# ruotianluo/ImageCaptioning.pytorch

Hardware: NVIDIA H100
Metric: captions/sec at beam=5 seq_len=20 (higher is better)
Workload: dtype f32 (fp32-grade: split-fp16 x3 tensor-core passes, fp32 accumulate)

## Files before the change

### imagecaptioning.pytorch_b200/csrc/beam.cu

```cuda
#include "common.cuh"
#include "kernels.cuh"

namespace capb200 {

namespace {

constexpr int MAXB = 16;

__device__ __forceinline__ double apply_penalty(int kind, float alpha, int length, double p) {
    if (kind == 1) return p / (pow(5.0 + length, (double)alpha) / pow(6.0, (double)alpha));
    if (kind == 2) return p / (double)length;
    return p;
}

__device__ __forceinline__ void select_step(const BeamState& s, int img, int t, int live, int kl, int row0, int hist0, const float* __restrict__ top_val,
                                            const int* __restrict__ top_idx, const int* pen, int n_pen, float lambda, int penalty_kind,
                                            float penalty_alpha, double* __restrict__ done_p) {
    const int lane = threadIdx.x;
    const int b = s.beam, T = s.T;
    const int ncand = live * kl;
    float cv[8];
    int cf[8];
#pragma unroll
    for (int u = 0; u < 8; ++u) {
// ... 74 lines not shown
            s.done_len[rec] = t + 1;
            s.done_raw[rec] = new_sum;
            done_p[rec] = apply_penalty(penalty_kind, penalty_alpha, t + 1, (double)new_sum);
            new_sum -= 1000.0f;
        }
        s.sums[(long)img * b + lane] = new_sum;
        s.tokens[(long)img * b + lane] = word;
        s.src_row[(long)img * b + lane] = row0 + parent;
    }
    if (lane == 0 && em != 0u) s.done_cnt[img] = cnt0 + __popc(em);
}

__global__ void __launch_bounds__(32) beam_step_kernel(BeamState s, int t, int live, const float* __restrict__ top_val,
                                                       const int* __restrict__ top_idx, int penalty_kind, float penalty_alpha,
                                                       double* __restrict__ done_p) {
    const int img = blockIdx.x;
    select_step(s, img, t, live, s.beam, img * live, img * live, top_val, top_idx, nullptr, 0, 0.f, penalty_kind, penalty_alpha, done_p);
}

__global__ void __launch_bounds__(32) diverse_beam_step_kernel(BeamState s, int G, int t, int k, const float* __restrict__ top_val,
                                                               const int* __restrict__ top_idx, float lambda, int rows_total, int penalty_kind,
                                                               float penalty_alpha, double* __restrict__ done_p) {
    const int i = blockIdx.x, lane = threadIdx.x;
    const int b = s.beam, T = s.T;
    __shared__ int sh_pen[MAXB];
    for (int g = 0; g < G && g <= t; ++g) {
        const int lt = t - g;
        if (lt >= T) continue;
        const int n_pen = g * b;
        __syncwarp();
        if (lane < n_pen) {
            const int pg = lane / b, j = lane - pg * b;
            const int last = min(t - pg, T - 1);
            const int* seq_pg = (last & 1) ? s.seq_a : s.seq_b;
            sh_pen[lane] = seq_pg[((long)(i * G + pg) * b + j) * T + lt];
        }
        __syncwarp();
        const int vimg = i * G + g;
        select_step(s, vimg, lt, lt == 0 ? 1 : b, k, vimg * b, g * rows_total + vimg * b, top_val, top_idx, sh_pen, n_pen, lambda, penalty_kind,
                    penalty_alpha, done_p);
    }
}

__global__ void __launch_bounds__(32) beam_finalize_kernel(BeamState s, int keep, const double* __restrict__ done_p, long long* __restrict__ out_seq,
                                                           int* __restrict__ out_len, float* __restrict__ out_p, float* __restrict__ out_raw,
                                                           int* __restrict__ out_hist) {
    const int img = blockIdx.x, lane = threadIdx.x;
    const int b = s.beam, T = s.T;
    const int cnt = s.done_cnt[img];
    const long base = (long)img * b * T;
    __shared__ unsigned char taken[MAXB * 64];
    for (int i = lane; i < cnt; i += 32) taken[i] = 0;
    __syncwarp();
    for (int k = 0; k < keep; ++k) {
        double bv = -INFINITY;
        int bi = 0x7fffffff;
        for (int i = lane; i < cnt; i += 32) {
            if (!taken[i]) {
                const double v = done_p[base + i];
                if (v > bv || (v == bv && i < bi)) { bv = v; bi = i; }
            }
// ... 16 lines not shown
            out_p[o] = (float)bv;
            out_raw[o] = s.done_raw[base + bi];
        }
        const int len = s.done_len[base + bi];
        for (int q = lane; q < T; q += 32) {
            out_seq[o * T + q] = (q < len) ? (long long)s.done_seq[(base + bi) * T + q] : 0;
            out_hist[o * T + q] = (q < len) ? s.done_hist[(base + bi) * T + q] : -1;
        }
        __syncwarp();
    }
}

__global__ void beam_edit_kernel(int rows, int k_in, int beam, int t, DecodeEdits ed, const int* __restrict__ prev_tokens,
                                 const float* __restrict__ val_in, const int* __restrict__ idx_in, float* __restrict__ val_out, int* __restrict__ idx_out,
                                 int first_beam, int first_group_rows, int first_group) {
    const int r = blockIdx.x * blockDim.x + threadIdx.x;
    if (r >= rows) return;
    if (first_beam > 0 && (r % first_beam) / first_group_rows == first_group) t = 0;
    float v[MAXB];
    int ix[MAXB];
    const int prev = (t > 0 && prev_tokens != nullptr) ? prev_tokens[r] : -1;
    bool prev_bad = false;
    if (t > 0 && ed.n_bad > 0)
        for (int i = 0; i < ed.n_bad; ++i) prev_bad |= (ed.bad[i] == prev);
    for (int k = 0; k < k_in; ++k) {
        float x = val_in[(long)r * k_in + k];
        const int w = idx_in[(long)r * k_in + k];
        if (ed.constraint && t > 0 && w == prev) x = -INFINITY;
        if (prev_bad && w == 0) x = -INFINITY;
        if (w == ed.unk_col) x -= 1000.0f;
        v[k] = x;
        ix[k] = w;
    }
    for (int j = 0; j < beam; ++j) {
        int best = j;
        for (int k = j + 1; k < k_in; ++k)
            if (v[k] > v[best] || (v[k] == v[best] && ix[k] < ix[best])) best = k;
        const float tv = v[j]; v[j] = v[best]; v[best] = tv;
        const int ti = ix[j]; ix[j] = ix[best]; ix[best] = ti;
        val_out[(long)r * beam + j] = v[j];
        idx_out[(long)r * beam + j] = ix[j];
    }
}

__global__ void scale_rows_kernel(float* __restrict__ x, long ld, int rows, int cols, float f, int skip_beam, int skip_group_rows, int skip_group) {
    const long total = (long)rows * cols;
    for (long i = blockIdx.x * (long)blockDim.x + threadIdx.x; i < total; i += (long)gridDim.x * blockDim.x) {
        const long r = i / cols, c = i % cols;
        if (skip_beam > 0 && (int)(r % skip_beam) / skip_group_rows == skip_group) continue;
        x[r * ld + c] *= f;
    }
}

__global__ void gather_rows_kernel(const float* __restrict__ slab, long step_stride, long ld_slab, const int* __restrict__ hist, int T, int V1,
                                   float* __restrict__ dst, const float2* __restrict__ stats, long stats_stride, const long long* __restrict__ seqs,
                                   DecodeEdits ed) {
    const long item = blockIdx.x;
    const int sidx = (int)(item % T);
    const int row = hist[item];
    float* d = dst + item * V1;
    if (row < 0) {
        for (int v = threadIdx.x; v < V1; v += blockDim.x) d[v] = 0.f;
        return;
    }
    auto apply_edits = [&]() {
        if (seqs == nullptr || !ed.any()) return;
        __syncthreads();
        if (threadIdx.x == 0) {
            const int prev = sidx > 0 ? (int)seqs[item - 1] : -1;
            if (ed.unk_col >= 0 && ed.unk_col < V1) d[ed.unk_col] -= 1000.0f;
            if (ed.constraint && prev >= 0 && prev < V1) d[prev] = -INFINITY;
// ... 35 lines not shown
        const float4* s4 = reinterpret_cast<const float4*>(src);
        float4* d4 = reinterpret_cast<float4*>(d);
        for (int v = threadIdx.x; v < V1 / 4; v += blockDim.x) d4[v] = __ldg(s4 + v);
    } else {
        for (int v = threadIdx.x; v < V1; v += blockDim.x) d[v] = src[v];
    }
    apply_edits();
}

}

int beam_edit_launch(int rows, int k_in, int beam, int t, const DecodeEdits& ed, const int* prev_tokens, const float* val_in, const int* idx_in,
                     float* val_out, int* idx_out, cudaStream_t stream, int first_beam, int first_group_rows, int first_group) {
    CAPB_REQUIRE(k_in >= beam && k_in <= MAXB, "beam_size + number of active decode edits must be <= 16");
    if (rows <= 0) return 0;
    beam_edit_kernel<<<cdiv(rows, 128), 128, 0, stream>>>(rows, k_in, beam, t, ed, prev_tokens, val_in, idx_in, val_out, idx_out, first_beam,
                                                          first_group_rows, first_group);
    CAPB_CHECK_CUDA(cudaGetLastError());
    return 0;
}

int scale_rows_launch(float* x, long ld, int rows, int cols, float factor, cudaStream_t stream, int skip_beam, int skip_group_rows, int skip_group) {
    if (rows <= 0 || cols <= 0) return 0;
    long blocks = ((long)rows * cols + 255) / 256;
    if (blocks > sm_count() * 16) blocks = sm_count() * 16;
    scale_rows_kernel<<<(int)blocks, 256, 0, stream>>>(x, ld, rows, cols, factor, skip_beam, skip_group_rows, skip_group);
    CAPB_CHECK_CUDA(cudaGetLastError());
    return 0;
}

int beam_step_launch(const BeamState& s, int t, int live, const float* top_val, const int* top_idx, int penalty_kind, float penalty_alpha,
                     cudaStream_t stream) {
    CAPB_REQUIRE(s.beam >= 1 && s.beam <= MAXB, "beam size 1..16");
    CAPB_REQUIRE(s.beam * s.T <= MAXB * 64, "beam*T record capacity");
    beam_step_kernel<<<s.B, 32, 0, stream>>>(s, t, live, top_val, top_idx, penalty_kind, penalty_alpha, s.done_p);
    CAPB_CHECK_CUDA(cudaGetLastError());
    return 0;
}

int diverse_beam_step_launch(const BeamState& s, int G, int t, int k, const float* top_val, const int* top_idx, float lambda, int rows_total,
                             int penalty_kind, float penalty_alpha, cudaStream_t stream) {
    CAPB_REQUIRE(G >= 2 && s.beam >= 1 && G * s.beam <= MAXB, "group_size * beams per group must be in 2..16");
    CAPB_REQUIRE(k >= s.beam && k <= MAXB && s.beam * k <= 256, "candidate list width");
    CAPB_REQUIRE(s.beam * s.T <= MAXB * 64, "beam*T record capacity");
    CAPB_REQUIRE(lambda >= 0.f, "diversity_lambda must be >= 0 (the candidate lists rely on the penalty only lowering values)");
    diverse_beam_step_kernel<<<s.B / G, 32, 0, stream>>>(s, G, t, k, top_val, top_idx, lambda, rows_total, penalty_kind, penalty_alpha, s.done_p);
    CAPB_CHECK_CUDA(cudaGetLastError());
    return 0;
}

int beam_finalize_launch(const BeamState& s, int keep, long long* out_seq, int* out_len, float* out_p, float* out_raw, int* out_hist,
                         cudaStream_t stream) {
    CAPB_REQUIRE(keep >= 1 && keep <= s.beam, "keep must be in 1..beam");
    beam_finalize_kernel<<<s.B, 32, 0, stream>>>(s, keep, s.done_p, out_seq, out_len, out_p, out_raw, out_hist);
    CAPB_CHECK_CUDA(cudaGetLastError());
    return 0;
}

int gather_logprob_rows_launch(const float* slab, long step_stride, long ld_slab, const int* hist, int nseq, int T, int V1, float* dst,
                               const float2* stats, long stats_stride, cudaStream_t stream, const long long* seqs, const DecodeEdits* ed) {
    if (nseq <= 0) return 0;
    gather_rows_kernel<<<nseq * T, 256, 0, stream>>>(slab, step_stride, ld_slab, hist, T, V1, dst, stats, stats_stride, seqs, ed ? *ed : DecodeEdits());
    CAPB_CHECK_CUDA(cudaGetLastError());
    return 0;
}

}
```

### imagecaptioning.pytorch_b200/csrc/common.cuh

```cuda
#pragma once
#include <atomic>
#include <cstdint>
#include <cstdio>
#include <cstring>
#include <string>
#include <cuda.h>
#include <cuda_fp16.h>
#include <cuda_runtime.h>

namespace capb200 {

void set_error(const std::string& msg);
#define CAPB_CHECK_CUDA(expr)                                                                          \
    do {                                                                                               \
        cudaError_t _e = (expr);                                                                       \
        if (_e != cudaSuccess) {                                                                       \
            capb200::set_error(std::string(#expr) + " failed: " + cudaGetErrorString(_e) + " at " +    \
                               __FILE__ + ":" + std::to_string(__LINE__));                            \
            return 1;                                                                                  \
        }                                                                                              \
    } while (0)
#define CAPB_REQUIRE(cond, msg)                                                                        \
    do {                                                                                               \
        if (!(cond)) {                                                                                 \
// ... 10 lines not shown
    if (cudaGetDevice(&dev) != cudaSuccess || dev < 0 || dev > 63) return true;
    const unsigned long long bit = 1ull << dev;
    return (mask.fetch_or(bit) & bit) == 0;
}

inline int sm_count() {
    static std::atomic<int> cache[64];
    int dev = 0;
    if (cudaGetDevice(&dev) != cudaSuccess || dev < 0 || dev > 63) dev = 0;
    int n = cache[dev].load();
    if (n == 0) {
        if (cudaDeviceGetAttribute(&n, cudaDevAttrMultiProcessorCount, dev) != cudaSuccess || n < 1) n = 132;
        cache[dev].store(n);
    }
    return n;
}

__device__ __forceinline__ void split_f32(float x, __half& hi, __half& lo) {
    hi = __float2half_rn(x);
    lo = __float2half_rn(x - __half2float(hi));
}

constexpr int kMaxSeg = 3;
struct GemmSeg {
    const float* A = nullptr;
    long lda = 0;
    const float* W = nullptr;
    long ldw = 0;
    const __half* A_hi = nullptr;
    const __half* A_lo = nullptr;
// ... 90 lines not shown
```

### imagecaptioning.pytorch_b200/csrc/engine_common.cuh

```cuda
#pragma once
#include <cstdio>
#include <cstdlib>
#include <cstring>

#include "../../include/capb200.h"
#include "common.cuh"
#include "kernels.cuh"
#include "nvtx.cuh"

struct capb200_cider_table {
    capb200::CiderTable* t = nullptr;
};

namespace capb200 {

struct Planes {
    __half* hi = nullptr;
    __half* lo = nullptr;
    long ld = 0;
};

struct Arena {
    char* base = nullptr;
    size_t off = 0;
// ... 235 lines not shown
            va.topk = edits ? k_in : beam; va.top_val = d.top_val; va.top_idx = d.top_idx;
            va.stats = d.slab_stats + (long)t * rows;
            if (vocab_step_launch(va, st)) return 1;
            const float* tv = d.top_val;
            const int* ti = d.top_idx;
            if (edits) {
                if (beam_edit_launch(nrows, k_in, beam, t, ed, d.tokens, d.top_val, d.top_idx, d.top_val_e, d.top_idx_e, st)) return 1;
                tv = d.top_val_e; ti = d.top_idx_e;
                *launches += 1;
            }
            if (beam_step_launch(s, t, live, tv, ti, penalty_kind, penalty_alpha, st)) return 1;
            *launches += 2;
        }
        return 0;
    };
    unsigned long long key[8] = {graph_key, (unsigned long long)B, (unsigned long long)beam, (unsigned long long)T, (unsigned long long)V1,
                                 (unsigned long long)penalty_kind, 0ull, (unsigned long long)reinterpret_cast<uintptr_t>(d.slab)};
    memcpy(&key[6], &penalty_alpha, sizeof(float));
    memcpy(reinterpret_cast<char*>(&key[6]) + 4, &temperature, sizeof(float));
    key[5] ^= ((unsigned long long)(ed.constraint & 1) << 8) ^ ((unsigned long long)(unsigned)(ed.unk_col + 1) << 16) ^ ((unsigned long long)ed.n_bad << 48);
    key[0] ^= (unsigned long long)reinterpret_cast<uintptr_t>(ed.bad) * 0x9E3779B97F4A7C15ull;
    d.last_edits = ed;
    d.last_stats = d.slab_stats;
    if (run_beam_loop(d, key, graph_key != 0, launches, st, run_loop)) return 1;
    CAPB_NVTX("capb200 beam finalize + log-prob rows");
    if (beam_finalize_launch(s, beam, d.rec_seq, d.rec_len, d.rec_p, d.rec_raw, d.rec_hist, st)) return 1;
    *launches += 1;
    if (keep == beam) {
        CAPB_CHECK_CUDA(cudaMemcpyAsync(seq, d.rec_seq, sizeof(long long) * B * beam * T, cudaMemcpyDeviceToDevice, st));
        if (seq_logprobs) {
            *launches += 1;
// ... 59 lines not shown
            va.topk = edits ? k_in : beam; va.top_val = d.top_val; va.top_idx = d.top_idx;
            va.stats = d.dbs_stats + (long)t * rows;
            if (vocab_step_launch(va, st)) return 1;
            const float* tv = d.top_val;
            const int* ti = d.top_idx;
            if (edits) {
                if (beam_edit_launch(rows, k_in, beam, t, ed, d.tokens, d.top_val, d.top_idx, d.top_val_e, d.top_idx_e, st, beam, bdash, t)) return 1;
                tv = d.top_val_e; ti = d.top_idx_e;
                *launches += 1;
            }
            if (diverse_beam_step_launch(s, G, t, beam, tv, ti, lambda, rows, penalty_kind, penalty_alpha, st)) return 1;
            *launches += 2;
        }
        return 0;
    };
    unsigned long long key[8] = {graph_key, (unsigned long long)B, (unsigned long long)beam, (unsigned long long)T, (unsigned long long)V1,
                                 (unsigned long long)penalty_kind, 0ull, (unsigned long long)reinterpret_cast<uintptr_t>(d.slab)};
    memcpy(&key[6], &penalty_alpha, sizeof(float));
    memcpy(reinterpret_cast<char*>(&key[6]) + 4, &temperature, sizeof(float));
    key[5] ^= ((unsigned long long)(ed.constraint & 1) << 8) ^ ((unsigned long long)(unsigned)(ed.unk_col + 1) << 16) ^ ((unsigned long long)ed.n_bad << 48);
    key[0] ^= (unsigned long long)reinterpret_cast<uintptr_t>(ed.bad) * 0x9E3779B97F4A7C15ull;
    unsigned lambda_bits = 0;
    memcpy(&lambda_bits, &lambda, sizeof(float));
    key[3] ^= (1ull << 63) ^ ((unsigned long long)G << 40);
    key[1] ^= (unsigned long long)lambda_bits << 32;
    key[4] ^= (unsigned long long)reinterpret_cast<uintptr_t>(d.dbs_stats) * 0x9E3779B97F4A7C15ull;
    key[2] ^= (unsigned long long)reinterpret_cast<uintptr_t>(d.dbs_done_cnt) << 8;
    if (run_beam_loop(d, key, graph_key != 0, launches, st, run_loop)) return 1;

    CAPB_NVTX("capb200 diverse beam finalize + log-prob rows");
    if (beam_finalize_launch(s, bdash, d.rec_seq, d.rec_len, d.rec_p, d.rec_raw, d.rec_hist, st)) return 1;
// ... 236 lines not shown
```

### imagecaptioning.pytorch_b200/csrc/gemm_tc.cu

```cuda
#include <cstdlib>
#include <cstring>

#include "common.cuh"
#include "ptx.cuh"

namespace capb200 {

namespace {

constexpr int BM = 128;
constexpr int BK = 64;
constexpr int kConsumers = 2;
constexpr int kThreads = 128 * (1 + kConsumers);

struct TcParams {
    CUtensorMap a_hi[kMaxSeg];
    CUtensorMap a_lo[kMaxSeg];
    CUtensorMap w_hi[kMaxSeg];
    CUtensorMap w_lo[kMaxSeg];
    int kblocks[kMaxSeg];
    int nseg;
    int M, N;
    float* C;
    long ldc;
// ... 360 lines not shown
    extern __shared__ uint8_t smem_raw[];
    uint8_t* smem = reinterpret_cast<uint8_t*>((reinterpret_cast<uintptr_t>(smem_raw) + 1023) & ~uintptr_t(1023));
    uint64_t* full_bar = reinterpret_cast<uint64_t*>(smem + Cfg::kStages * Cfg::kStageBytes);
    uint64_t* empty_bar = full_bar + Cfg::kStages;
    uint64_t* turn_bar = empty_bar + Cfg::kStages;

    const int wg = threadIdx.x >> 7;
    const int n_tiles = p.tiles_m * p.tiles_n;

    if (threadIdx.x == 0) {
        init_ring<PASSES>(p, full_bar, empty_bar, Cfg::kStages, 1);
        for (int c = 0; c < kConsumers; ++c) ptx::mbar_init(&turn_bar[c], 1);
        ptx::fence_mbar_init();
    }
    __syncthreads();
    if (threadIdx.x == 0) CAPB_TRACE(0);

    if (wg == 0) {
        ptx::setmaxnreg_dec<40>();
        if (threadIdx.x == 0) {
            int stage = 0;
            uint32_t phase = 0;
            for (int t = blockIdx.x; t < n_tiles; t += gridDim.x) {
                const int m0 = (t % p.tiles_m) * BM;
                const int n0 = (t / p.tiles_m) * BN;
                for (int s = 0; s < p.nseg; ++s) {
                    for (int kb = 0; kb < p.kblocks[s]; ++kb) {
                        ptx::mbar_wait(&empty_bar[stage], phase ^ 1);
                        fill_stage<Cfg>(p, smem + stage * Cfg::kStageBytes, &full_bar[stage], s, kb, m0, n0);
                        if (++stage == Cfg::kStages) { stage = 0; phase ^= 1; }
// ... 44 lines not shown
__global__ void __launch_bounds__(kThreads, 1) gemm_tc256_kernel(const __grid_constant__ TcParams p) {
    using Cfg = TcCfg<BN, PASSES, 2 * BM>;
    extern __shared__ uint8_t smem_raw[];
    uint8_t* smem = reinterpret_cast<uint8_t*>((reinterpret_cast<uintptr_t>(smem_raw) + 1023) & ~uintptr_t(1023));
    uint64_t* full_bar = reinterpret_cast<uint64_t*>(smem + Cfg::kStages * Cfg::kStageBytes);
    uint64_t* empty_bar = full_bar + Cfg::kStages;

    const int wg = threadIdx.x >> 7;
    const int n_tiles = p.tiles_m * p.tiles_n;

    if (threadIdx.x == 0) {
        init_ring<PASSES>(p, full_bar, empty_bar, Cfg::kStages, kConsumers);
        ptx::fence_mbar_init();
    }
    __syncthreads();
    if (threadIdx.x == 0) CAPB_TRACE(0);

    if (wg == 0) {
        ptx::setmaxnreg_dec<40>();
        if (threadIdx.x == 0) {
            int stage = 0;
            uint32_t phase = 0;
            for (int t = blockIdx.x; t < n_tiles; t += gridDim.x) {
                const int m0 = (t % p.tiles_m) * Cfg::kTileM;
                const int n0 = (t / p.tiles_m) * BN;
                for (int s = 0; s < p.nseg; ++s) {
                    for (int kb = 0; kb < p.kblocks[s]; ++kb) {
                        ptx::mbar_wait(&empty_bar[stage], phase ^ 1);
                        fill_stage<Cfg>(p, smem + stage * Cfg::kStageBytes, &full_bar[stage], s, kb, m0, n0);
                        if (++stage == Cfg::kStages) { stage = 0; phase ^= 1; }
// ... 69 lines not shown
template <int BN, int PASSES, int EPI, bool TRACE, int TM>
int launch_cfg(const TcParams& prm, cudaStream_t stream) {
    using Cfg = TcCfg<BN, PASSES, TM>;
    void (*kernel)(TcParams);
    if constexpr (TM == BM) kernel = gemm_tc_kernel<BN, PASSES, EPI, TRACE>;
    else kernel = gemm_tc256_kernel<BN, PASSES, EPI, TRACE>;
    static std::atomic<unsigned long long> attr_set{0};
    if (first_use_on_device(attr_set)) {
        CAPB_CHECK_CUDA(cudaFuncSetAttribute(kernel, cudaFuncAttributeMaxDynamicSharedMemorySize, Cfg::kSmemBytes));
    }
    TcParams prm2 = prm;
    prm2.tiles_n = cdiv(prm.N, BN);
    prm2.tiles_m = cdiv(prm.M, TM);
    const int n_tiles = prm2.tiles_n * prm2.tiles_m;
    const int sms = sm_count();
    kernel<<<n_tiles < sms ? n_tiles : sms, kThreads, Cfg::kSmemBytes, stream>>>(prm2);
    CAPB_CHECK_CUDA(cudaGetLastError());
    return 0;
}

template <int EPI, int TM>
int launch_width(int bn, int passes, const TcParams& prm, cudaStream_t stream) {
    if (prm.trace != nullptr) {
        if (bn == 160) return launch_cfg<160, 3, EPI, true, TM>(prm, stream);
        if constexpr (TM == BM) if (bn == 64) return launch_cfg<64, 3, EPI, true, TM>(prm, stream);
        return launch_cfg<128, 3, EPI, true, TM>(prm, stream);
    }
    if (bn == 160) return passes == 3 ? launch_cfg<160, 3, EPI, false, TM>(prm, stream) : launch_cfg<160, 1, EPI, false, TM>(prm, stream);
    if constexpr (TM == BM) {
        if (bn == 64) return passes == 3 ? launch_cfg<64, 3, EPI, false, TM>(prm, stream) : launch_cfg<64, 1, EPI, false, TM>(prm, stream);
    }
    return passes == 3 ? launch_cfg<128, 3, EPI, false, TM>(prm, stream) : launch_cfg<128, 1, EPI, false, TM>(prm, stream);
// ... 114 lines not shown
```

### imagecaptioning.pytorch_b200/csrc/pointwise.cu

```cuda
#include "common.cuh"
#include "kernels.cuh"

namespace capb200 {

static int pw_blocks(long total) {
    long b = (total + 255) / 256;
    return (int)(b > sm_count() * 8 ? sm_count() * 8 : b);
}

namespace {

__device__ __forceinline__ float sigmoidf_(float x) { return fast_sigmoid(x); }

__device__ __forceinline__ void store_act(const ActView& o, long row, int col, float v) {
    o.f[row * o.ld + col] = v;
    if (o.hi != nullptr) {
        __half h, l;
        split_f32(v, h, l);
        o.hi[row * o.ld + col] = h;
        o.lo[row * o.ld + col] = l;
    }
}

__global__ void state_gather_embed_kernel(int rows, const int* __restrict__ tokens, const int* __restrict__ src_row,
                                          const float* __restrict__ emb, long ld_emb, int E, int relu, ActView xt,
                                          int H, int nstate, StateCopy sc0, StateCopy sc1) {
    const int r = blockIdx.x;
    if (r >= rows) return;
    const int tok = tokens[r];
    const float* e = emb + (long)tok * ld_emb;
    for (int c = threadIdx.x; c < E; c += blockDim.x) {
        float v = __ldg(e + c);
        if (relu) v = fmaxf(v, 0.f);
        store_act(xt, r, c, v);
    }
    const int src = src_row ? src_row[r] : r;
    const bool vec = (H & 3) == 0 && (sc0.ld_src & 3) == 0 && (sc0.dst.ld & 3) == 0 && (nstate < 2 || ((sc1.ld_src & 3) == 0 && (sc1.dst.ld & 3) == 0));
    if (vec) {
        for (int c4 = threadIdx.x; c4 < (H >> 2); c4 += blockDim.x) {
            float4 v0 = make_float4(0.f, 0.f, 0.f, 0.f), v1 = v0;
            if (src >= 0) {
// ... 112 lines not shown
    extern __shared__ float s_ah[];
    constexpr int AP = NA * 32;
    float* s_w = s_ah + ATT_JB * AP;
    constexpr float kC = 2.885390081777927f;
    const int img = blockIdx.y;
    const int warp = threadIdx.x >> 5, lane = threadIdx.x & 31;
    const int r = blockIdx.x * ATT_SW + warp;
    const float alpha_b = __ldg(alpha_b_ptr);
    float pv[NA];
    const bool live = r < R;
    const float* pr = p_att + ((long)img * R + (live ? r : 0)) * ld_pa;
    for (int i = threadIdx.x; i < AP; i += ATT_SW * 32) s_w[i] = (i < A) ? __ldg(alpha_w + i) : 0.f;
    __syncthreads();
    float wsum = 0.f;
#pragma unroll
    for (int k = 0; k < NA; ++k) {
        const int a = (NA % 4 == 0) ? 128 * (k >> 2) + 4 * lane + (k & 3) : lane + 32 * k;
        pv[k] = (live && a < A) ? __ldg(pr + a) * kC : 0.f;
        wsum += s_w[a];
    }
    for (int j0 = 0; j0 < rpi; j0 += ATT_JB) {
        const int nj = min(ATT_JB, rpi - j0);
        __syncthreads();
        for (int i = threadIdx.x; i < nj * AP; i += ATT_SW * 32) {
            const int j = i / AP, a = i - j * AP;
            s_ah[i] = (a < A) ? att_h[((long)img * rpi + j0 + j) * ld_ah + a] * kC : 0.f;
        }
        __syncthreads();
        if (live) {
            float part[ATT_JB];
#pragma unroll
            for (int j = 0; j < ATT_JB; ++j) {
                part[j] = 0.f;
                if (j < nj) {
// ... 34 lines not shown
#pragma unroll
            for (int j = 0; j < ATT_JB; ++j) {
                float v = part[j];
#pragma unroll
                for (int o = 16; o > 0; o >>= 1) v += __shfl_xor_sync(0xffffffffu, v, o);
                if (lane == 0 && j < nj) score[((long)img * rpi + j0 + j) * R + r] = v + alpha_b;
            }
        }
    }
}

constexpr int ATT_CT = 256;
__global__ void __launch_bounds__(ATT_CT) att_combine_kernel(int rpi, int R, int H, const float* __restrict__ score, const float* __restrict__ att,
                                                             long ld_at, const float* __restrict__ mask, long ld_mask, ActView out,
                                                             float* __restrict__ alpha_out) {
    extern __shared__ float s_w[];
    const int img = blockIdx.x;
    const int c = blockIdx.y * ATT_CT + threadIdx.x;
    const int warp = threadIdx.x >> 5, lane = threadIdx.x & 31;
    for (int j0 = 0; j0 < rpi; j0 += ATT_JB) {
        const int nj = min(ATT_JB, rpi - j0);
        __syncthreads();
        if (warp < nj) {
            const float* sc = score + ((long)img * rpi + j0 + warp) * R;
            float* w = s_w + warp * R;
            float mx = -INFINITY;
            for (int r = lane; r < R; r += 32) mx = fmaxf(mx, sc[r]);
#pragma unroll
            for (int o = 16; o > 0; o >>= 1) mx = fmaxf(mx, __shfl_xor_sync(0xffffffffu, mx, o));
            float sum = 0.f;
// ... 42 lines not shown
        if (out_flat.hi) { __half h, l; split_f32(v, h, l); out_flat.hi[i] = h; out_flat.lo[i] = l; }
    }
}

}

int relu_copy_launch(const float* x, long n, ActView out_flat, cudaStream_t stream) {
    relu_copy_kernel<<<pw_blocks(n), 256, 0, stream>>>(x, n, out_flat);
    CAPB_CHECK_CUDA(cudaGetLastError());
    return 0;
}

int state_gather_embed_launch(int rows, const int* tokens, const int* src_row, const float* emb, long ld_emb, int E, int relu,
                              ActView xt, int H, int nstate, StateCopy sc0, StateCopy sc1, cudaStream_t stream) {
    if (rows <= 0) return 0;
    state_gather_embed_kernel<<<rows, 256, 0, stream>>>(rows, tokens, src_row, emb, ld_emb, E, relu, xt, H, nstate, sc0, sc1);
    CAPB_CHECK_CUDA(cudaGetLastError());
    return 0;
}


int lstm_pointwise_launch(int rows, int H, const float* gates, long ld_g, const int* src_row, const float* c_prev, long ld_cp,
                          float* c_out, long ld_co, ActView h_out, const float* gather_bias, long ld_gb, const int* gather_idx,
                          cudaStream_t stream) {
    if (rows <= 0) return 0;
    lstm_pointwise_kernel<<<pw_blocks((long)rows * H), 256, 0, stream>>>(rows, H, gates, ld_g, src_row, c_prev, ld_cp, c_out, ld_co, h_out,
                                                                          gather_bias, ld_gb, gather_idx);
    CAPB_CHECK_CUDA(cudaGetLastError());
    return 0;
}

int lstm_ln_launch(int rows, int H, const float* gates, long ld_g, const float* c_prev, long ld_cp, float* c_out, long ld_co, float* h_out, long ld_h,
// ... 9 lines not shown
                            float* c_out, long ld_co, ActView h_out, cudaStream_t stream) {
    if (rows <= 0) return 0;
    maxout_pointwise_kernel<<<pw_blocks((long)rows * H), 256, 0, stream>>>(rows, H, sums, ld_s, src_row, c_prev, ld_cp, c_out, ld_co, h_out);
    CAPB_CHECK_CUDA(cudaGetLastError());
    return 0;
}

int additive_attention_launch(int n_images, int rpi, int R, int A, int H, const float* att_h, long ld_ah, const float* p_att, long ld_pa,
                              const float* att, long ld_at, const float* mask, long ld_mask, const float* alpha_w, const float* alpha_b,
                              float* score_scratch, ActView out, cudaStream_t stream, float* alpha_out) {
    if (n_images <= 0 || rpi <= 0) return 0;
    CAPB_REQUIRE(A <= 1024, "attention: att_hid_size above 1024");
    CAPB_REQUIRE(score_scratch != nullptr, "attention: score scratch missing");
    const int na = cdiv(A, 32);
    dim3 sgrid(cdiv(R, ATT_SW), n_images);
#define CAPB_ATT_CASE(NA_)                                                                                                             \
    att_score_kernel<NA_><<<sgrid, ATT_SW * 32, sizeof(float) * (ATT_JB + 1) * NA_ * 32, stream>>>(rpi, R, A, att_h, ld_ah, p_att, ld_pa, alpha_w, \
                                                                                               alpha_b, score_scratch)
    if (na <= 2) CAPB_ATT_CASE(2);
    else if (na <= 4) CAPB_ATT_CASE(4);
    else if (na <= 8) CAPB_ATT_CASE(8);
    else if (na <= 16) CAPB_ATT_CASE(16);
    else CAPB_ATT_CASE(32);
#undef CAPB_ATT_CASE
    CAPB_CHECK_CUDA(cudaGetLastError());
    const size_t smem = sizeof(float) * (size_t)ATT_JB * R;
    CAPB_REQUIRE(smem <= 48 * 1024, "attention: too many regions");
    dim3 grid(n_images, cdiv(H, ATT_CT));
    att_combine_kernel<<<grid, ATT_CT, smem, stream>>>(rpi, R, H, score_scratch, att, ld_at, mask, ld_mask, out, alpha_out);
    CAPB_CHECK_CUDA(cudaGetLastError());
    return 0;
}

}
```

### imagecaptioning.pytorch_b200/csrc/vocab.cu

```cuda
#include <cstdlib>

#include "common.cuh"
#include "kernels.cuh"
#include "ptx.cuh"

namespace capb200 {

static __device__ unsigned long long g_vocab_seed_salt = 0ull;
int dropout_salt_set_vocab(unsigned long long salt, cudaStream_t st) {
    return cudaMemcpyToSymbolAsync(g_vocab_seed_salt, &salt, sizeof(salt), 0, cudaMemcpyHostToDevice, st) == cudaSuccess ? 0 : 1;
}

namespace {

constexpr int VT = 256;

template <int NT = VT>
__device__ __forceinline__ float block_max(float v, float* scratch) {
#pragma unroll
    for (int o = 16; o > 0; o >>= 1) v = fmaxf(v, __shfl_xor_sync(0xffffffffu, v, o));
    __syncthreads();
    if ((threadIdx.x & 31) == 0) scratch[threadIdx.x >> 5] = v;
    __syncthreads();
    float r = scratch[0];
// ... 205 lines not shown
            }
            float ov;
            block_argmax<NT>(bv, bi, s_red, s_idx, ov, tok);
        }
        __syncthreads();
        if (threadIdx.x == 0) {
            if (a.unfinished) a.unfinished[r] = (tok != 0) ? 1 : 0;
            if (a.tokens_out) a.tokens_out[r] = tok;
            if (a.seq_out) a.seq_out[(long)r * a.ld_seq + a.t] = tok;
            if (a.picked_lp) a.picked_lp[(long)r * a.ld_picked] = row[tok];
        }
    }
}

__global__ void __launch_bounds__(VT) vocab_stats_kernel(const VocabStepArgs a) {
    __shared__ float s_red[VT / 32];
    __shared__ int s_idx[VT / 32];
    const int r = blockIdx.x;
    const int V1 = a.V1;
    const float* g = a.logits + (long)r * a.ld;
    const bool vec = ((V1 & 3) == 0) && ((a.ld & 3) == 0) && ((reinterpret_cast<uintptr_t>(a.logits) & 15) == 0);
    float mx = -INFINITY;
    if (vec) {
        const float4* g4 = reinterpret_cast<const float4*>(g);
        for (int v = threadIdx.x; v < V1 / 4; v += VT) { const float4 x = g4[v]; mx = fmaxf(mx, fmaxf(fmaxf(x.x, x.y), fmaxf(x.z, x.w))); }
    } else {
        for (int v = threadIdx.x; v < V1; v += VT) mx = fmaxf(mx, g[v]);
    }
    mx = block_max(mx, s_red);
    float t0v = -INFINITY, t1v = -INFINITY;
// ... 56 lines not shown
__device__ __forceinline__ void online_raise(float& part, float& m, float& mL, float m4) {
    const float nL = m4 * 1.4426950408889634f;
    float sc;
    asm("ex2.approx.ftz.f32 %0, %1;" : "=f"(sc) : "f"(mL - nL));
    part = (m == -INFINITY) ? 0.f : part * sc;
    m = m4;
    mL = nL;
}
__device__ __forceinline__ float online_finish(float part, float m, float mL, float mx) {
    float sc;
    asm("ex2.approx.ftz.f32 %0, %1;" : "=f"(sc) : "f"(fmaf(-mx, 1.4426950408889634f, mL)));
    return (m == -INFINITY) ? 0.f : part * sc;
}

__global__ void __launch_bounds__(VT) vocab_stats_online_kernel(const VocabStepArgs a) {
    __shared__ float s_red[VT / 32];
    __shared__ int s_idx[VT / 32];
    const int r = blockIdx.x;
    const int n4 = a.V1 >> 2;
    const float4* g4 = reinterpret_cast<const float4*>(a.logits + (long)r * a.ld);
    constexpr float kL2E = 1.4426950408889634f;
    float t0v = -INFINITY, t1v = -INFINITY;
    int t0i = 0x7fffffff, t1i = 0x7fffffff;
    float m = -INFINITY, mL = -INFINITY, part = 0.f;
    for (int v = threadIdx.x; v < n4; v += VT) {
        const float4 x = g4[v];
        const float m4 = fmaxf(fmaxf(x.x, x.y), fmaxf(x.z, x.w));
        if (m4 > m) {
            online_raise(part, m, mL, m4);
        }
// ... 75 lines not shown
    }
    __syncthreads();
    if ((threadIdx.x & 31) == 0) { sval[threadIdx.x >> 5] = v; sidx[threadIdx.x >> 5] = i; }
    __syncthreads();
    out_v = sval[0];
    out_i = sidx[0];
#pragma unroll
    for (int w = 1; w < VT2 / 32; ++w) {
        const float ov = sval[w];
        const int oi = sidx[w];
        if (ov > out_v || (ov == out_v && oi < out_i)) { out_v = ov; out_i = oi; }
    }
}

__global__ void __launch_bounds__(VT2) vocab_stats_online128_kernel(const VocabStepArgs a) {
    __shared__ float s_red[VT2 / 32];
    __shared__ int s_idx[VT2 / 32];
    const int r = blockIdx.x;
    const int n4 = a.V1 >> 2;
    const float4* g4 = reinterpret_cast<const float4*>(a.logits + (long)r * a.ld);
    constexpr float kL2E = 1.4426950408889634f;
    float t0v = -INFINITY, t1v = -INFINITY;
    int t0i = 0x7fffffff, t1i = 0x7fffffff;
    float m = -INFINITY, mL = -INFINITY, part = 0.f;
    auto consume = [&](const float4 x, int v) {
        const float m4 = fmaxf(fmaxf(x.x, x.y), fmaxf(x.z, x.w));
        if (m4 > m) {
            online_raise(part, m, mL, m4);
        }
        float e0, e1, e2, e3;
// ... 44 lines not shown
                    const float4 x = g4[w];
                    consider(x.x, 4 * w); consider(x.y, 4 * w + 1); consider(x.z, 4 * w + 2); consider(x.w, 4 * w + 3);
                }
            }
        }
        if (threadIdx.x == 0) {
            const float lp = (ov - mx) - lsum;
            a.top_val[(long)r * a.topk + k] = a.row_twice(r) ? (lp - m2) - l2 : lp;
            a.top_idx[(long)r * a.topk + k] = oi;
        }
    }
}

template <int NV>
__global__ void __launch_bounds__(VT) vocab_stats_reg_kernel(const VocabStepArgs a) {
    __shared__ float s_red[VT / 32];
    __shared__ int s_idx[VT / 32];
    const int r = blockIdx.x;
    const int n4 = a.V1 >> 2;
    const float4* g4 = reinterpret_cast<const float4*>(a.logits + (long)r * a.ld);
    float4 xs[NV];
#pragma unroll
    for (int i = 0; i < NV; ++i) {
        const int v = threadIdx.x + i * VT;
        xs[i] = v < n4 ? g4[v] : make_float4(-INFINITY, -INFINITY, -INFINITY, -INFINITY);
    }
    float mx = -INFINITY;
#pragma unroll
    for (int i = 0; i < NV; ++i) mx = fmaxf(mx, fmaxf(fmaxf(xs[i].x, xs[i].y), fmaxf(xs[i].z, xs[i].w)));
    mx = block_max(mx, s_red);
// ... 35 lines not shown
                for (int i = 0; i < NV; ++i) {
                    const int v = 4 * (threadIdx.x + i * VT);
                    if (v < a.V1) { consider(xs[i].x, v); consider(xs[i].y, v + 1); consider(xs[i].z, v + 2); consider(xs[i].w, v + 3); }
                }
            }
        }
        if (threadIdx.x == 0) {
            const float lp = (ov - mx) - lsum;
            a.top_val[(long)r * a.topk + k] = a.row_twice(r) ? (lp - m2) - l2 : lp;
            a.top_idx[(long)r * a.topk + k] = oi;
        }
    }
}

__global__ void __launch_bounds__(VT) vocab_stats_stream_kernel(const VocabStepArgs a) {
    extern __shared__ __align__(16) unsigned char vs_smem[];
    __shared__ float s_red[VT / 32];
    __shared__ int s_idx[VT / 32];
    __shared__ __align__(8) uint64_t bar[2];
    const int V1 = a.V1, n4 = V1 >> 2;
    const uint32_t row_bytes = (uint32_t)V1 * 4u;
    float* buf0 = reinterpret_cast<float*>(vs_smem);
    float* buf1 = buf0 + V1;
    if (threadIdx.x == 0) {
        ptx::mbar_init(&bar[0], 1);
        ptx::mbar_init(&bar[1], 1);
        ptx::fence_mbar_init();
    }
    __syncthreads();
    int r = blockIdx.x;
// ... 113 lines not shown
    }
}

}

int vocab_step_launch(const VocabStepArgs& a, cudaStream_t stream) {
    if (a.rows <= 0) return 0;
    CAPB_REQUIRE(a.topk <= 16, "beam size up to 16");
    if (a.stats != nullptr) {
        CAPB_REQUIRE(a.select == 0 && a.topk > 0, "stats mode is the beam-search epilogue");
        const bool vec = ((a.V1 & 3) == 0) && ((a.ld & 3) == 0) && ((reinterpret_cast<uintptr_t>(a.logits) & 15) == 0);
        const size_t stream_smem = sizeof(float) * 2 * (size_t)a.V1;
        static const char* variant = getenv("CAPB200_VOCAB_STATS");
        const char vsel = variant ? variant[0] : 'o';
        if (vec && vsel == 'o' && !(variant && variant[1] == '2')) {
            vocab_stats_online128_kernel<<<a.rows, VT2, 0, stream>>>(a);
        } else if (vec && vsel == 'o') {
            vocab_stats_online_kernel<<<a.rows, VT, 0, stream>>>(a);
        } else if (vec && vsel == 's' && stream_smem <= 100 * 1024) {
            static std::atomic<unsigned long long> configured{0};
            if (first_use_on_device(configured)) {
                CAPB_CHECK_CUDA(cudaFuncSetAttribute(vocab_stats_stream_kernel, cudaFuncAttributeMaxDynamicSharedMemorySize, (int)(100 * 1024)));
            }
            const int grid = a.rows < 2 * sm_count() ? a.rows : 2 * sm_count();
            vocab_stats_stream_kernel<<<grid, VT, stream_smem, stream>>>(a);
        } else if (vec && vsel == 'r' && a.V1 <= VT * 4 * 10) {
            vocab_stats_reg_kernel<10><<<a.rows, VT, 0, stream>>>(a);
        } else {
            vocab_stats_kernel<<<a.rows, VT, 0, stream>>>(a);
        }
        CAPB_CHECK_CUDA(cudaGetLastError());
        return 0;
    }
    const size_t smem = sizeof(float) * (size_t)a.V1;
    CAPB_REQUIRE(smem <= 200 * 1024, "vocabulary larger than 51200 entries needs the multi-pass variant");
    static std::atomic<unsigned long long> configured{0};
    if (first_use_on_device(configured)) {
        CAPB_CHECK_CUDA(cudaFuncSetAttribute(vocab_step_kernel<2>, cudaFuncAttributeMaxDynamicSharedMemorySize, (int)(200 * 1024)));
        CAPB_CHECK_CUDA(cudaFuncSetAttribute(vocab_step_kernel<8>, cudaFuncAttributeMaxDynamicSharedMemorySize, (int)(200 * 1024)));
        CAPB_CHECK_CUDA(cudaFuncSetAttribute(vocab_step_kernel<16>, cudaFuncAttributeMaxDynamicSharedMemorySize, (int)(200 * 1024)));
    }
    if (a.topk <= 2 && a.select != 0 && a.rows <= 2 * sm_count()) {
        static std::atomic<unsigned long long> configured2{0};
        if (first_use_on_device(configured2)) {
// ... 28 lines not shown
```

Before: 23870.

## Enable programmatic dependent launch across decode-step kernels

Launches the beam, attention, vocab, pointwise and GEMM kernels with the programmatic stream serialization attribute, adding griddepcontrol wait and launch-dependents calls at kernel entry. The next kernel's launch and prologue (barrier init, smem setup, attention weight sum) can then overlap the tail of the previous kernel in the many small per-step launches. The graph cache key now includes the PDL setting, and an environment variable can turn it off. The risk is a memory ordering error if a kernel touches predecessor outputs before its wait.

Result: faster. 24380, median of 6 (+2.1%).

```diff
diff --git a/imagecaptioning.pytorch_b200/csrc/beam.cu b/imagecaptioning.pytorch_b200/csrc/beam.cu
--- a/imagecaptioning.pytorch_b200/csrc/beam.cu
+++ b/imagecaptioning.pytorch_b200/csrc/beam.cu
@@ -112,6 +112,7 @@
 __global__ void __launch_bounds__(32) beam_step_kernel(BeamState s, int t, int live, const float* __restrict__ top_val,
                                                        const int* __restrict__ top_idx, int penalty_kind, float penalty_alpha,
                                                        double* __restrict__ done_p) {
+    pdl_enter();
     const int img = blockIdx.x;
     select_step(s, img, t, live, s.beam, img * live, img * live, top_val, top_idx, nullptr, 0, 0.f, penalty_kind, penalty_alpha, done_p);
 }
@@ -119,6 +120,7 @@
 __global__ void __launch_bounds__(32) diverse_beam_step_kernel(BeamState s, int G, int t, int k, const float* __restrict__ top_val,
                                                                const int* __restrict__ top_idx, float lambda, int rows_total, int penalty_kind,
                                                                float penalty_alpha, double* __restrict__ done_p) {
+    pdl_enter();
     const int i = blockIdx.x, lane = threadIdx.x;
     const int b = s.beam, T = s.T;
     __shared__ int sh_pen[MAXB];
@@ -143,6 +145,7 @@
 __global__ void __launch_bounds__(32) beam_finalize_kernel(BeamState s, int keep, const double* __restrict__ done_p, long long* __restrict__ out_seq,
                                                            int* __restrict__ out_len, float* __restrict__ out_p, float* __restrict__ out_raw,
                                                            int* __restrict__ out_hist) {
+    pdl_enter();
     const int img = blockIdx.x, lane = threadIdx.x;
     const int b = s.beam, T = s.T;
     const int cnt = s.done_cnt[img];
@@ -189,6 +192,7 @@
 __global__ void beam_edit_kernel(int rows, int k_in, int beam, int t, DecodeEdits ed, const int* __restrict__ prev_tokens,
                                  const float* __restrict__ val_in, const int* __restrict__ idx_in, float* __restrict__ val_out, int* __restrict__ idx_out,
                                  int first_beam, int first_group_rows, int first_group) {
+    pdl_enter();
     const int r = blockIdx.x * blockDim.x + threadIdx.x;
     if (r >= rows) return;
     if (first_beam > 0 && (r % first_beam) / first_group_rows == first_group) t = 0;
@@ -219,6 +223,7 @@
 }
 
 __global__ void scale_rows_kernel(float* __restrict__ x, long ld, int rows, int cols, float f, int skip_beam, int skip_group_rows, int skip_group) {
+    pdl_enter();
     const long total = (long)rows * cols;
     for (long i = blockIdx.x * (long)blockDim.x + threadIdx.x; i < total; i += (long)gridDim.x * blockDim.x) {
         const long r = i / cols, c = i % cols;
@@ -230,6 +235,7 @@
 __global__ void gather_rows_kernel(const float* __restrict__ slab, long step_stride, long ld_slab, const int* __restrict__ hist, int T, int V1,
                                    float* __restrict__ dst, const float2* __restrict__ stats, long stats_stride, const long long* __restrict__ seqs,
                                    DecodeEdits ed) {
+    pdl_enter();
     const long item = blockIdx.x;
     const int sidx = (int)(item % T);
     const int row = hist[item];
@@ -295,9 +301,8 @@
                      float* val_out, int* idx_out, cudaStream_t stream, int first_beam, int first_group_rows, int first_group) {
     CAPB_REQUIRE(k_in >= beam && k_in <= MAXB, "beam_size + number of active decode edits must be <= 16");
     if (rows <= 0) return 0;
-    beam_edit_kernel<<<cdiv(rows, 128), 128, 0, stream>>>(rows, k_in, beam, t, ed, prev_tokens, val_in, idx_in, val_out, idx_out, first_beam,
-                                                          first_group_rows, first_group);
-    CAPB_CHECK_CUDA(cudaGetLastError());
+    CAPB_CHECK_CUDA(launch_pdl(beam_edit_kernel, dim3(cdiv(rows, 128)), dim3(128), 0, stream, rows, k_in, beam, t, ed, prev_tokens, val_in, idx_in,
+                               val_out, idx_out, first_beam, first_group_rows, first_group));
     return 0;
 }
 
@@ -305,8 +310,8 @@
     if (rows <= 0 || cols <= 0) return 0;
     long blocks = ((long)rows * cols + 255) / 256;
     if (blocks > sm_count() * 16) blocks = sm_count() * 16;
-    scale_rows_kernel<<<(int)blocks, 256, 0, stream>>>(x, ld, rows, cols, factor, skip_beam, skip_group_rows, skip_group);
-    CAPB_CHECK_CUDA(cudaGetLastError());
+    CAPB_CHECK_CUDA(launch_pdl(scale_rows_kernel, dim3((int)blocks), dim3(256), 0, stream, x, ld, rows, cols, factor, skip_beam, skip_group_rows,
+                               skip_group));
     return 0;
 }
 
@@ -314,8 +319,7 @@
                      cudaStream_t stream) {
     CAPB_REQUIRE(s.beam >= 1 && s.beam <= MAXB, "beam size 1..16");
     CAPB_REQUIRE(s.beam * s.T <= MAXB * 64, "beam*T record capacity");
-    beam_step_kernel<<<s.B, 32, 0, stream>>>(s, t, live, top_val, top_idx, penalty_kind, penalty_alpha, s.done_p);
-    CAPB_CHECK_CUDA(cudaGetLastError());
+    CAPB_CHECK_CUDA(launch_pdl(beam_step_kernel, dim3(s.B), dim3(32), 0, stream, s, t, live, top_val, top_idx, penalty_kind, penalty_alpha, s.done_p));
     return 0;
 }
 
@@ -325,25 +329,24 @@
     CAPB_REQUIRE(k >= s.beam && k <= MAXB && s.beam * k <= 256, "candidate list width");
     CAPB_REQUIRE(s.beam * s.T <= MAXB * 64, "beam*T record capacity");
     CAPB_REQUIRE(lambda >= 0.f, "diversity_lambda must be >= 0 (the candidate lists rely on the penalty only lowering values)");
-    diverse_beam_step_kernel<<<s.B / G, 32, 0, stream>>>(s, G, t, k, top_val, top_idx, lambda, rows_total, penalty_kind, penalty_alpha, s.done_p);
-    CAPB_CHECK_CUDA(cudaGetLastError());
+    CAPB_CHECK_CUDA(launch_pdl(diverse_beam_step_kernel, dim3(s.B / G), dim3(32), 0, stream, s, G, t, k, top_val, top_idx, lambda, rows_total,
+                               penalty_kind, penalty_alpha, s.done_p));
     return 0;
 }
 
 int beam_finalize_launch(const BeamState& s, int keep, long long* out_seq, int* out_len, float* out_p, float* out_raw, int* out_hist,
                          cudaStream_t stream) {
     CAPB_REQUIRE(keep >= 1 && keep <= s.beam, "keep must be in 1..beam");
-    beam_finalize_kernel<<<s.B, 32, 0, stream>>>(s, keep, s.done_p, out_seq, out_len, out_p, out_raw, out_hist);
-    CAPB_CHECK_CUDA(cudaGetLastError());
+    CAPB_CHECK_CUDA(launch_pdl(beam_finalize_kernel, dim3(s.B), dim3(32), 0, stream, s, keep, s.done_p, out_seq, out_len, out_p, out_raw, out_hist));
     return 0;
 }
 
 int gather_logprob_rows_launch(const float* slab, long step_stride, long ld_slab, const int* hist, int nseq, int T, int V1, float* dst,
                                const float2* stats, long stats_stride, cudaStream_t stream, const long long* seqs, const DecodeEdits* ed) {
     if (nseq <= 0) return 0;
-    gather_rows_kernel<<<nseq * T, 256, 0, stream>>>(slab, step_stride, ld_slab, hist, T, V1, dst, stats, stats_stride, seqs, ed ? *ed : DecodeEdits());
-    CAPB_CHECK_CUDA(cudaGetLastError());
-    return 0;
-}
-
-}
+    CAPB_CHECK_CUDA(launch_pdl(gather_rows_kernel, dim3(nseq * T), dim3(256), 0, stream, slab, step_stride, ld_slab, hist, T, V1, dst, stats,
+                               stats_stride, seqs, ed ? *ed : DecodeEdits()));
+    return 0;
+}
+
+}
diff --git a/imagecaptioning.pytorch_b200/csrc/common.cuh b/imagecaptioning.pytorch_b200/csrc/common.cuh
--- a/imagecaptioning.pytorch_b200/csrc/common.cuh
+++ b/imagecaptioning.pytorch_b200/csrc/common.cuh
@@ -2,8 +2,10 @@
 #include <atomic>
 #include <cstdint>
 #include <cstdio>
+#include <cstdlib>
 #include <cstring>
 #include <string>
+#include <utility>
 #include <cuda.h>
 #include <cuda_fp16.h>
 #include <cuda_runtime.h>
@@ -48,6 +50,33 @@
         cache[dev].store(n);
     }
     return n;
+}
+
+__device__ __forceinline__ void pdl_wait() { asm volatile("griddepcontrol.wait;" ::: "memory"); }
+__device__ __forceinline__ void pdl_launch_dependents() { asm volatile("griddepcontrol.launch_dependents;" ::: "memory"); }
+__device__ __forceinline__ void pdl_enter() {
+    pdl_wait();
+    pdl_launch_dependents();
+}
+
+inline bool pdl_enabled() {
+    const char* v = getenv("CAPB200_NO_PDL");
+    return v == nullptr || strcmp(v, "1") != 0;
+}
+
+template <typename... KArgs, typename... Args>
+cudaError_t launch_pdl(void (*kernel)(KArgs...), dim3 grid, dim3 block, size_t smem, cudaStream_t stream, Args&&... args) {
+    cudaLaunchAttribute attr[1];
+    attr[0].id = cudaLaunchAttributeProgrammaticStreamSerialization;
+    attr[0].val.programmaticStreamSerializationAllowed = 1;
+    cudaLaunchConfig_t cfg = {};
+    cfg.gridDim = grid;
+    cfg.blockDim = block;
+    cfg.dynamicSmemBytes = smem;
+    cfg.stream = stream;
+    cfg.attrs = attr;
+    cfg.numAttrs = pdl_enabled() ? 1 : 0;
+    return cudaLaunchKernelEx(&cfg, kernel, std::forward<Args>(args)...);
 }
 
 __device__ __forceinline__ void split_f32(float x, __half& hi, __half& lo) {
diff --git a/imagecaptioning.pytorch_b200/csrc/engine_common.cuh b/imagecaptioning.pytorch_b200/csrc/engine_common.cuh
--- a/imagecaptioning.pytorch_b200/csrc/engine_common.cuh
+++ b/imagecaptioning.pytorch_b200/csrc/engine_common.cuh
@@ -273,7 +273,8 @@
         }
         return 0;
     };
-    unsigned long long key[8] = {graph_key, (unsigned long long)B, (unsigned long long)beam, (unsigned long long)T, (unsigned long long)V1,
+    unsigned long long key[8] = {graph_key, (unsigned long long)(unsigned)B | ((unsigned long long)pdl_enabled() << 32), (unsigned long long)beam,
+                                 (unsigned long long)T, (unsigned long long)V1,
                                  (unsigned long long)penalty_kind, 0ull, (unsigned long long)reinterpret_cast<uintptr_t>(d.slab)};
     memcpy(&key[6], &penalty_alpha, sizeof(float));
     memcpy(reinterpret_cast<char*>(&key[6]) + 4, &temperature, sizeof(float));
@@ -363,7 +364,8 @@
         }
         return 0;
     };
-    unsigned long long key[8] = {graph_key, (unsigned long long)B, (unsigned long long)beam, (unsigned long long)T, (unsigned long long)V1,
+    unsigned long long key[8] = {graph_key, (unsigned long long)(unsigned)B | ((unsigned long long)pdl_enabled() << 32), (unsigned long long)beam,
+                                 (unsigned long long)T, (unsigned long long)V1,
                                  (unsigned long long)penalty_kind, 0ull, (unsigned long long)reinterpret_cast<uintptr_t>(d.slab)};
     memcpy(&key[6], &penalty_alpha, sizeof(float));
     memcpy(reinterpret_cast<char*>(&key[6]) + 4, &temperature, sizeof(float));
diff --git a/imagecaptioning.pytorch_b200/csrc/gemm_tc.cu b/imagecaptioning.pytorch_b200/csrc/gemm_tc.cu
--- a/imagecaptioning.pytorch_b200/csrc/gemm_tc.cu
+++ b/imagecaptioning.pytorch_b200/csrc/gemm_tc.cu
@@ -398,6 +398,7 @@
         ptx::fence_mbar_init();
     }
     __syncthreads();
+    pdl_wait();
     if (threadIdx.x == 0) CAPB_TRACE(0);
 
     if (wg == 0) {
@@ -472,6 +473,7 @@
         ptx::fence_mbar_init();
     }
     __syncthreads();
+    pdl_wait();
     if (threadIdx.x == 0) CAPB_TRACE(0);
 
     if (wg == 0) {
@@ -571,8 +573,7 @@
     prm2.tiles_m = cdiv(prm.M, TM);
     const int n_tiles = prm2.tiles_n * prm2.tiles_m;
     const int sms = sm_count();
-    kernel<<<n_tiles < sms ? n_tiles : sms, kThreads, Cfg::kSmemBytes, stream>>>(prm2);
-    CAPB_CHECK_CUDA(cudaGetLastError());
+    CAPB_CHECK_CUDA(launch_pdl(kernel, dim3(n_tiles < sms ? n_tiles : sms), dim3(kThreads), Cfg::kSmemBytes, stream, prm2));
     return 0;
 }
 
diff --git a/imagecaptioning.pytorch_b200/csrc/pointwise.cu b/imagecaptioning.pytorch_b200/csrc/pointwise.cu
--- a/imagecaptioning.pytorch_b200/csrc/pointwise.cu
+++ b/imagecaptioning.pytorch_b200/csrc/pointwise.cu
@@ -25,6 +25,7 @@
 __global__ void state_gather_embed_kernel(int rows, const int* __restrict__ tokens, const int* __restrict__ src_row,
                                           const float* __restrict__ emb, long ld_emb, int E, int relu, ActView xt,
                                           int H, int nstate, StateCopy sc0, StateCopy sc1) {
+    pdl_enter();
     const int r = blockIdx.x;
     if (r >= rows) return;
     const int tok = tokens[r];
@@ -167,10 +168,12 @@
     __syncthreads();
     float wsum = 0.f;
 #pragma unroll
+    for (int k = 0; k < NA; ++k) wsum += s_w[(NA % 4 == 0) ? 128 * (k >> 2) + 4 * lane + (k & 3) : lane + 32 * k];
+    pdl_enter();
+#pragma unroll
     for (int k = 0; k < NA; ++k) {
         const int a = (NA % 4 == 0) ? 128 * (k >> 2) + 4 * lane + (k & 3) : lane + 32 * k;
         pv[k] = (live && a < A) ? __ldg(pr + a) * kC : 0.f;
-        wsum += s_w[a];
     }
     for (int j0 = 0; j0 < rpi; j0 += ATT_JB) {
         const int nj = min(ATT_JB, rpi - j0);
@@ -235,6 +238,7 @@
 __global__ void __launch_bounds__(ATT_CT) att_combine_kernel(int rpi, int R, int H, const float* __restrict__ score, const float* __restrict__ att,
                                                              long ld_at, const float* __restrict__ mask, long ld_mask, ActView out,
                                                              float* __restrict__ alpha_out) {
+    pdl_enter();
     extern __shared__ float s_w[];
     const int img = blockIdx.x;
     const int c = blockIdx.y * ATT_CT + threadIdx.x;
@@ -307,8 +311,8 @@
 int state_gather_embed_launch(int rows, const int* tokens, const int* src_row, const float* emb, long ld_emb, int E, int relu,
                               ActView xt, int H, int nstate, StateCopy sc0, StateCopy sc1, cudaStream_t stream) {
     if (rows <= 0) return 0;
-    state_gather_embed_kernel<<<rows, 256, 0, stream>>>(rows, tokens, src_row, emb, ld_emb, E, relu, xt, H, nstate, sc0, sc1);
-    CAPB_CHECK_CUDA(cudaGetLastError());
+    CAPB_CHECK_CUDA(launch_pdl(state_gather_embed_kernel, dim3(rows), dim3(256), 0, stream, rows, tokens, src_row, emb, ld_emb, E, relu, xt, H,
+                               nstate, sc0, sc1));
     return 0;
 }
 
@@ -348,22 +352,17 @@
     CAPB_REQUIRE(score_scratch != nullptr, "attention: score scratch missing");
     const int na = cdiv(A, 32);
     dim3 sgrid(cdiv(R, ATT_SW), n_images);
-#define CAPB_ATT_CASE(NA_)                                                                                                             \
-    att_score_kernel<NA_><<<sgrid, ATT_SW * 32, sizeof(float) * (ATT_JB + 1) * NA_ * 32, stream>>>(rpi, R, A, att_h, ld_ah, p_att, ld_pa, alpha_w, \
-                                                                                               alpha_b, score_scratch)
-    if (na <= 2) CAPB_ATT_CASE(2);
-    else if (na <= 4) CAPB_ATT_CASE(4);
-    else if (na <= 8) CAPB_ATT_CASE(8);
-    else if (na <= 16) CAPB_ATT_CASE(16);
-    else CAPB_ATT_CASE(32);
-#undef CAPB_ATT_CASE
-    CAPB_CHECK_CUDA(cudaGetLastError());
+    void (*score_kernel)(int, int, int, const float*, long, const float*, long, const float*, const float*, float*) =
+        na <= 2 ? att_score_kernel<2> : na <= 4 ? att_score_kernel<4> : na <= 8 ? att_score_kernel<8> : na <= 16 ? att_score_kernel<16> : att_score_kernel<32>;
+    const int na_p2 = na <= 2 ? 2 : na <= 4 ? 4 : na <= 8 ? 8 : na <= 16 ? 16 : 32;
+    CAPB_CHECK_CUDA(launch_pdl(score_kernel, sgrid, dim3(ATT_SW * 32), sizeof(float) * (ATT_JB + 1) * na_p2 * 32, stream, rpi, R, A, att_h, ld_ah,
+                               p_att, ld_pa, alpha_w, alpha_b, score_scratch));
     const size_t smem = sizeof(float) * (size_t)ATT_JB * R;
     CAPB_REQUIRE(smem <= 48 * 1024, "attention: too many regions");
     dim3 grid(n_images, cdiv(H, ATT_CT));
-    att_combine_kernel<<<grid, ATT_CT, smem, stream>>>(rpi, R, H, score_scratch, att, ld_at, mask, ld_mask, out, alpha_out);
-    CAPB_CHECK_CUDA(cudaGetLastError());
-    return 0;
-}
-
-}
+    CAPB_CHECK_CUDA(launch_pdl(att_combine_kernel, grid, dim3(ATT_CT), smem, stream, rpi, R, H, score_scratch, att, ld_at, mask, ld_mask, out,
+                               alpha_out));
+    return 0;
+}
+
+}
diff --git a/imagecaptioning.pytorch_b200/csrc/vocab.cu b/imagecaptioning.pytorch_b200/csrc/vocab.cu
--- a/imagecaptioning.pytorch_b200/csrc/vocab.cu
+++ b/imagecaptioning.pytorch_b200/csrc/vocab.cu
@@ -243,6 +243,7 @@
 }
 
 __global__ void __launch_bounds__(VT) vocab_stats_kernel(const VocabStepArgs a) {
+    pdl_enter();
     __shared__ float s_red[VT / 32];
     __shared__ int s_idx[VT / 32];
     const int r = blockIdx.x;
@@ -329,6 +330,7 @@
 }
 
 __global__ void __launch_bounds__(VT) vocab_stats_online_kernel(const VocabStepArgs a) {
+    pdl_enter();
     __shared__ float s_red[VT / 32];
     __shared__ int s_idx[VT / 32];
     const int r = blockIdx.x;
@@ -434,6 +436,7 @@
 }
 
 __global__ void __launch_bounds__(VT2) vocab_stats_online128_kernel(const VocabStepArgs a) {
+    pdl_enter();
     __shared__ float s_red[VT2 / 32];
     __shared__ int s_idx[VT2 / 32];
     const int r = blockIdx.x;
@@ -508,6 +511,7 @@
 
 template <int NV>
 __global__ void __launch_bounds__(VT) vocab_stats_reg_kernel(const VocabStepArgs a) {
+    pdl_enter();
     __shared__ float s_red[VT / 32];
     __shared__ int s_idx[VT / 32];
     const int r = blockIdx.x;
@@ -573,6 +577,7 @@
 }
 
 __global__ void __launch_bounds__(VT) vocab_stats_stream_kernel(const VocabStepArgs a) {
+    pdl_enter();
     extern __shared__ __align__(16) unsigned char vs_smem[];
     __shared__ float s_red[VT / 32];
     __shared__ int s_idx[VT / 32];
@@ -716,20 +721,20 @@
         static const char* variant = getenv("CAPB200_VOCAB_STATS");
         const char vsel = variant ? variant[0] : 'o';
         if (vec && vsel == 'o' && !(variant && variant[1] == '2')) {
-            vocab_stats_online128_kernel<<<a.rows, VT2, 0, stream>>>(a);
+            CAPB_CHECK_CUDA(launch_pdl(vocab_stats_online128_kernel, dim3(a.rows), dim3(VT2), 0, stream, a));
         } else if (vec && vsel == 'o') {
-            vocab_stats_online_kernel<<<a.rows, VT, 0, stream>>>(a);
+            CAPB_CHECK_CUDA(launch_pdl(vocab_stats_online_kernel, dim3(a.rows), dim3(VT), 0, stream, a));
         } else if (vec && vsel == 's' && stream_smem <= 100 * 1024) {
             static std::atomic<unsigned long long> configured{0};
             if (first_use_on_device(configured)) {
                 CAPB_CHECK_CUDA(cudaFuncSetAttribute(vocab_stats_stream_kernel, cudaFuncAttributeMaxDynamicSharedMemorySize, (int)(100 * 1024)));
             }
             const int grid = a.rows < 2 * sm_count() ? a.rows : 2 * sm_count();
-            vocab_stats_stream_kernel<<<grid, VT, stream_smem, stream>>>(a);
+            CAPB_CHECK_CUDA(launch_pdl(vocab_stats_stream_kernel, dim3(grid), dim3(VT), stream_smem, stream, a));
         } else if (vec && vsel == 'r' && a.V1 <= VT * 4 * 10) {
-            vocab_stats_reg_kernel<10><<<a.rows, VT, 0, stream>>>(a);
+            CAPB_CHECK_CUDA(launch_pdl(vocab_stats_reg_kernel<10>, dim3(a.rows), dim3(VT), 0, stream, a));
         } else {
-            vocab_stats_kernel<<<a.rows, VT, 0, stream>>>(a);
+            CAPB_CHECK_CUDA(launch_pdl(vocab_stats_kernel, dim3(a.rows), dim3(VT), 0, stream, a));
         }
         CAPB_CHECK_CUDA(cudaGetLastError());
         return 0;
```
